# the3cloud/zktls

Hardware: AMD Instinct MI355X
Metric: trace-cells/s (higher is better)
Workload: dtype u32

## Files before the change

### include/zkhip.h

```cpp
#ifndef ZKHIP_H
#define ZKHIP_H
#include <stddef.h>
#include <stdint.h>

#ifdef __cplusplus
extern "C" {
#endif

#define ZKHIP_VERSION 100

typedef enum {
    ZKHIP_OK = 0,
    ZKHIP_ERR_INVALID = -1,
    ZKHIP_ERR_NO_DEVICE = -2,
    ZKHIP_ERR_HIP = -3,
    ZKHIP_ERR_NOMEM = -4,
    ZKHIP_ERR_BUFFER = -5,
    ZKHIP_ERR_VERIFY = -6,
    ZKHIP_ERR_INTERNAL = -7
} zkhip_status;

typedef struct zkhip_ctx zkhip_ctx;

typedef struct {
// ... 12 lines not shown

int zkhip_version(void);
const char* zkhip_last_error(void);
int zkhip_device_count(void);
int zkhip_ctx_create(int device, void* stream, zkhip_ctx** out);
void zkhip_ctx_destroy(zkhip_ctx* ctx);
int zkhip_ctx_sync(zkhip_ctx* ctx);
int zkhip_set_wait_mode(int blocking, int device);
void* zkhip_ctx_stream(zkhip_ctx* ctx);

int zkhip_malloc(zkhip_ctx* ctx, size_t bytes, void** d_ptr);
int zkhip_free(zkhip_ctx* ctx, void* d_ptr);
int zkhip_memcpy_h2d(zkhip_ctx* ctx, void* d_dst, const void* h_src, size_t bytes);
int zkhip_memcpy_d2h(zkhip_ctx* ctx, void* h_dst, const void* d_src, size_t bytes);
int zkhip_to_monty(zkhip_ctx* ctx, const uint32_t* d_in, uint32_t* d_out, size_t n);
int zkhip_from_monty(zkhip_ctx* ctx, const uint32_t* d_in, uint32_t* d_out, size_t n);

int zkhip_fill_uniform(zkhip_ctx* ctx, uint64_t seed, int log_n, uint32_t width,
                       uint32_t* d_out, size_t ld);
int zkhip_gen_trace(zkhip_ctx* ctx, uint64_t seed, uint64_t shard, int log_n, uint32_t width,
                    uint32_t* d_out, size_t ld);

int zkhip_gen_trace_logup(zkhip_ctx* ctx, uint64_t seed, uint64_t shard, int log_n, uint32_t width,
                          int pairs, uint32_t* d_out, size_t ld);

int zkhip_gen_trace_logup_cross(zkhip_ctx* ctx, uint64_t seed, uint64_t shard, uint64_t partner_shard, int log_n, uint32_t width,
                                uint32_t partner_width, int pairs, uint32_t* d_out, size_t ld);

int zkhip_dft(zkhip_ctx* ctx, const uint32_t* d_in, size_t in_ld, uint32_t* d_out, size_t out_ld,
              int log_n, uint32_t width, int inverse, int bitrev_out);
int zkhip_coset_lde(zkhip_ctx* ctx, const uint32_t* d_in, size_t in_ld, uint32_t* d_out,
                    size_t out_ld, int log_n, uint32_t width, int log_blowup, uint32_t shift);
int zkhip_ctx_set_lde_fusion(zkhip_ctx* ctx, int on);

int zkhip_commit(zkhip_ctx* ctx, const uint32_t* d_trace, size_t ld, int log_n, uint32_t width, int log_blowup,
                 int hash_width, uint32_t* d_lde, uint32_t* d_tree, uint32_t root[8]);

int zkhip_poseidon2_permute(zkhip_ctx* ctx, uint32_t* d_states, size_t count);
int zkhip_hash_rows(zkhip_ctx* ctx, const uint32_t* const* d_mats, const size_t* lds,
                    const uint32_t* widths, int nmats, size_t height, uint32_t* d_digests);
int zkhip_merkle_commit(zkhip_ctx* ctx, const uint32_t* const* d_mats, const size_t* lds,
                        const uint32_t* widths, int nmats, int log_h, uint32_t* d_tree);

int zkhip_merkle_commit_mixed(zkhip_ctx* ctx, const uint32_t* const* d_mats, const size_t* lds,
                              const uint32_t* widths, const int* log_heights, int nmats, uint32_t* d_tree);


int zkhip_quotient_values(zkhip_ctx* ctx, const uint32_t* d_lde, size_t ld, int log_n,
                          uint32_t width, const uint32_t alpha[4] ,
                          uint32_t* d_out);
int zkhip_perm_trace(zkhip_ctx* ctx, const uint32_t* d_trace, size_t ld, int log_n, uint32_t width, int pairs,
                     const uint32_t gamma[4], const uint32_t beta[4], uint32_t* d_out);
int zkhip_open_at(zkhip_ctx* ctx, const uint32_t* d_lde, size_t ld, int log_n, int log_blowup,
                  uint32_t width, const uint32_t* z, int npoints, uint32_t* h_out);
int zkhip_fri_fold(zkhip_ctx* ctx, const uint32_t* d_in, int log_h,
                   const uint32_t beta[4] , uint32_t* d_out);

int zkhip_fri_fold_k(zkhip_ctx* ctx, const uint32_t* d_in, int log_h, int log_arity,
                     const uint32_t beta[4] , uint32_t* d_out);

size_t zkhip_proof_size(int log_n, uint32_t width, const zkhip_params* prm, size_t n_public);
int zkhip_prove_shard(zkhip_ctx* ctx, const uint32_t* d_trace, size_t ld, int log_n,
                      uint32_t width, const uint32_t* public_values, size_t n_public,
                      const zkhip_params* prm, uint8_t* proof, size_t cap, size_t* len);
int zkhip_prove_shard_host(zkhip_ctx* ctx, const uint32_t* h_trace, int log_n, uint32_t width,
                           const uint32_t* public_values, size_t n_public, const zkhip_params* prm,
// ... 222 lines not shown
```

### zktls_amd/_lib.py

```python
import ctypes as C
import os

import numpy as np

P = 2013265921
_HERE = os.path.dirname(os.path.abspath(__file__))
LIB_PATH = os.path.join(_HERE, "libzkhip.so")

u32p = C.POINTER(C.c_uint32)
u8p = C.POINTER(C.c_uint8)

EXPORTS = [
    "zkhip_version", "zkhip_last_error", "zkhip_device_count", "zkhip_ctx_create", "zkhip_ctx_destroy",
    "zkhip_ctx_sync", "zkhip_ctx_set_lde_fusion", "zkhip_ctx_stream", "zkhip_malloc", "zkhip_free", "zkhip_memcpy_h2d",
    "zkhip_memcpy_d2h", "zkhip_to_monty", "zkhip_from_monty", "zkhip_fill_uniform", "zkhip_gen_trace",
    "zkhip_gen_trace_logup", "zkhip_gen_trace_logup_cross", "zkhip_perm_trace",
    "zkhip_dft", "zkhip_coset_lde", "zkhip_ntt_pass", "zkhip_poseidon2_permute", "zkhip_hash_rows",
    "zkhip_merkle_commit", "zkhip_merkle_commit_mixed", "zkhip_merkle_commit_p24_colmajor", "zkhip_batch_interpolate_colmajor", "zkhip_batch_expand_colmajor", "zkhip_quotient_values", "zkhip_open_at", "zkhip_fri_fold", "zkhip_fri_fold_k",
    "zkhip_commit", "zkhip_proof_size", "zkhip_prove_shard", "zkhip_prove_shard_host", "zkhip_prove_shards", "zkhip_prove_shards_multi", "zkhip_shard_device", "zkhip_release_cached_contexts", "zkhip_prove_segment", "zkhip_verify_shard", "zkhip_last_prove_debug",
    "zkhip_chips_proof_size", "zkhip_prove_chips", "zkhip_verify_chips", "zkhip_request_digest",
    "zkhip_eltwise_add", "zkhip_eltwise_copy", "zkhip_eltwise_zeroize", "zkhip_eltwise_sum_ext", "zkhip_zk_shift", "zkhip_mix_poly_coeffs",
    "zkhip_batch_evaluate_any", "zkhip_gather_sample", "zkhip_scatter", "zkhip_prefix_products_ext", "zkhip_hash_rows_sha256",
    "zkhip_hash_fold_sha256", "zkhip_merkle_commit_sha256_colmajor",
    "zkhip_bincode_size", "zkhip_proof_to_bincode", "zkhip_proof_from_bincode",
    "zkhip_chips_bincode_size", "zkhip_chips_proof_to_bincode", "zkhip_chips_proof_from_bincode",
    "zkhip_load_poseidon2_params", "zkhip_reset_poseidon2_params", "zkhip_poseidon2_params_name",
    "zkhip_air_validate", "zkhip_air_digest", "zkhip_air_synthetic", "zkhip_proof_size_air", "zkhip_prove_shard_air", "zkhip_verify_shard_air",
    "zkhip_quotient_values_air",
    "zkhip_chips_proof_size_air", "zkhip_prove_chips_air", "zkhip_verify_chips_air",
    "zkhip_prove_shards_air_multi", "zkhip_selftest_host_simd", "zkhip_host_permutation_ns", "zkhip_host_simd", "zkhip_recursion_witnesses_on_host", "zkhip_machine_proof_size", "zkhip_prove_machine", "zkhip_verify_machine", "zkhip_range_table",
    "zkhip_machine_setup", "zkhip_machine_key_destroy", "zkhip_machine_proof_size_keyed", "zkhip_prove_machine_keyed", "zkhip_verify_machine_keyed", "zkhip_prove_machine_keyed_at",
    "zkhip_sha256_setup", "zkhip_sha256_machine_proof_size", "zkhip_prove_sha256_machine", "zkhip_verify_sha256_machine", "zkhip_prove_transcripts", "zkhip_prove_transcripts_air", "zkhip_sha256_machine_describe", "zkhip_machine_verifier_setup", "zkhip_machine_verifier_key_host", "zkhip_machine_verifier_proof_size", "zkhip_prove_machine_verifier", "zkhip_prove_shard_tree", "zkhip_verify_machine_recursive", "zkhip_machine_verifier_describe", "zkhip_machine_verifier_host_tables", "zkhip_sha256_compress_setup", "zkhip_sha256_compress_key_host", "zkhip_sha256_compressed_proof_size", "zkhip_prove_sha256_compressed", "zkhip_verify_sha256_compressed", "zkhip_set_wait_mode", "zkhip_set_lockstep", "zkhip_lockstep_stats", "zkhip_lockstep_stack_high_water", "zkhip_set_fri_graph", "zkhip_shard_verifier_setup", "zkhip_shard_verifier_proof_size", "zkhip_shard_verifier_max_proofs", "zkhip_prove_shard_verifier", "zkhip_prove_shard_verifier_batch", "zkhip_verify_shard_recursive", "zkhip_shard_verifier_describe", "zkhip_shard_verifier_key_host", "zkhip_machine_key_host", "zkhip_shard_verifier_setup_air", "zkhip_shard_verifier_key_host_air", "zkhip_shard_verifier_max_proofs_air", "zkhip_shard_verifier_proof_size_air", "zkhip_prove_shard_verifier_air", "zkhip_verify_shard_recursive_air", "zkhip_shard_verifier_describe_air", "zkhip_poseidon2_params_generation", "zkhip_selftest_lockstep",
    "zkhip_sha256_air_chained", "zkhip_sha256_gen_trace_chained", "zkhip_sha256_sharded_count", "zkhip_sha256_shard_proof_size", "zkhip_prove_sha256_sharded",
    "zkhip_verify_sha256_sharded",
    "zkhip_fri_view_shard", "zkhip_fri_chip_width", "zkhip_fri_chip_air",
    
    "zkhip_fri_view_path_words", "zkhip_fri_view_shard_paths", "zkhip_fri_view_transcript", "zkhip_fri_layers_chip_air", "zkhip_p2chip_air_fri_layers",
    
    "zkhip_fri_transcript_chip_air", "zkhip_p2chip_air_fri_transcript",
    
    "zkhip_fri_indices_program", "zkhip_fri_indices_key", "zkhip_fri_indices_proof_size", "zkhip_prove_fri_indices", "zkhip_verify_fri_indices",
    "zkhip_prove_fri_indices_batch", "zkhip_fri_view_all",
    "zkhip_p2chip_air", "zkhip_p2chip_gen_merkle_trace", "zkhip_merkle_paths_proof_size", "zkhip_prove_merkle_paths", "zkhip_verify_merkle_paths",
    "zkhip_p24chip_air", "zkhip_p24chip_gen_merkle_trace", "zkhip_merkle_paths_p24_proof_size", "zkhip_prove_merkle_paths_p24", "zkhip_verify_merkle_paths_p24",
    "zkhip_sha256_air", "zkhip_sha256_digest", "zkhip_sha256_pad", "zkhip_sha256_padding_publics", "zkhip_sha256_gen_trace", "zkhip_sha256_proof_size", "zkhip_prove_sha256", "zkhip_verify_sha256",
]

# ... 39 lines not shown
                ("n_public", C.c_size_t), ("proof", u8p), ("proof_cap", C.c_size_t), ("proof_len", C.c_size_t), ("status", C.c_int32)]


class ProveDebug(C.Structure):
    _fields_ = [
        ("trace_root", C.c_uint32 * 8),
        ("quotient_root", C.c_uint32 * 8),
        ("alpha", C.c_uint32 * 4),
        ("zeta", C.c_uint32 * 4),
        ("fri_alpha", C.c_uint32 * 4),
        ("pow_witness", C.c_uint32),
    ]


_LIB = None


def load():
    global _LIB
    if _LIB is not None:
        return _LIB
    if not os.path.exists(LIB_PATH):
        raise ImportError("libzkhip.so not built: run `python -c 'import __graft_entry__ as g; g.build()'` "
                          "(zktls_amd has no CPU fallback)")
    L = C.CDLL(LIB_PATH)
    L.zkhip_last_error.restype = C.c_char_p
    L.zkhip_ctx_stream.restype = C.c_void_p
    L.zkhip_ctx_stream.argtypes = [C.c_void_p]
    L.zkhip_ctx_create.argtypes = [C.c_int, C.c_void_p, C.POINTER(C.c_void_p)]
    L.zkhip_ctx_destroy.argtypes = [C.c_void_p]
    L.zkhip_ctx_destroy.restype = None
    L.zkhip_ctx_sync.argtypes = [C.c_void_p]
    L.zkhip_ctx_set_lde_fusion.argtypes = [C.c_void_p, C.c_int]
    L.zkhip_malloc.argtypes = [C.c_void_p, C.c_size_t, C.POINTER(C.c_void_p)]
    L.zkhip_free.argtypes = [C.c_void_p, C.c_void_p]
    L.zkhip_memcpy_h2d.argtypes = [C.c_void_p, C.c_void_p, C.c_void_p, C.c_size_t]
    L.zkhip_memcpy_d2h.argtypes = [C.c_void_p, C.c_void_p, C.c_void_p, C.c_size_t]
    L.zkhip_to_monty.argtypes = [C.c_void_p, C.c_void_p, C.c_void_p, C.c_size_t]
    L.zkhip_from_monty.argtypes = [C.c_void_p, C.c_void_p, C.c_void_p, C.c_size_t]
    L.zkhip_fill_uniform.argtypes = [C.c_void_p, C.c_uint64, C.c_int, C.c_uint32, C.c_void_p, C.c_size_t]
    L.zkhip_gen_trace.argtypes = [C.c_void_p, C.c_uint64, C.c_uint64, C.c_int, C.c_uint32, C.c_void_p, C.c_size_t]
    L.zkhip_gen_trace_logup.argtypes = [C.c_void_p, C.c_uint64, C.c_uint64, C.c_int, C.c_uint32, C.c_int, C.c_void_p, C.c_size_t]
    L.zkhip_perm_trace.argtypes = [C.c_void_p, C.c_void_p, C.c_size_t, C.c_int, C.c_uint32, C.c_int, u32p, u32p, C.c_void_p]
    L.zkhip_dft.argtypes = [C.c_void_p, C.c_void_p, C.c_size_t, C.c_void_p, C.c_size_t, C.c_int, C.c_uint32, C.c_int, C.c_int]
    L.zkhip_coset_lde.argtypes = [C.c_void_p, C.c_void_p, C.c_size_t, C.c_void_p, C.c_size_t, C.c_int, C.c_uint32, C.c_int, C.c_uint32]
    L.zkhip_ntt_pass.argtypes = [C.c_void_p, C.c_void_p, C.c_void_p, C.c_size_t, C.c_int, C.c_uint32, C.c_int]
    L.zkhip_poseidon2_permute.argtypes = [C.c_void_p, C.c_void_p, C.c_size_t]
    L.zkhip_hash_rows.argtypes = [C.c_void_p, C.POINTER(C.c_void_p), C.POINTER(C.c_size_t), C.POINTER(C.c_uint32), C.c_int, C.c_size_t, C.c_void_p]
    L.zkhip_merkle_commit.argtypes = [C.c_void_p, C.POINTER(C.c_void_p), C.POINTER(C.c_size_t), C.POINTER(C.c_uint32), C.c_int, C.c_int, C.c_void_p]
    L.zkhip_merkle_commit_mixed.argtypes = [C.c_void_p, C.POINTER(C.c_void_p), C.POINTER(C.c_size_t), C.POINTER(C.c_uint32), C.POINTER(C.c_int), C.c_int, C.c_void_p]
    L.zkhip_merkle_commit_p24_colmajor.argtypes = [C.c_void_p, C.c_void_p, C.c_uint32, C.c_int, C.c_void_p]
    L.zkhip_batch_interpolate_colmajor.argtypes = [C.c_void_p, C.c_void_p, C.c_void_p, C.c_uint32, C.c_int]
    L.zkhip_batch_expand_colmajor.argtypes = [C.c_void_p, C.c_void_p, C.c_void_p, C.c_uint32, C.c_int, C.c_int, C.c_uint32]
    L.zkhip_quotient_values.argtypes = [C.c_void_p, C.c_void_p, C.c_size_t, C.c_int, C.c_uint32, u32p, C.c_void_p]
    L.zkhip_open_at.argtypes = [C.c_void_p, C.c_void_p, C.c_size_t, C.c_int, C.c_int, C.c_uint32, u32p, C.c_int, u32p]
    L.zkhip_fri_fold.argtypes = [C.c_void_p, C.c_void_p, C.c_int, u32p, C.c_void_p]
    L.zkhip_fri_fold_k.argtypes = [C.c_void_p, C.c_void_p, C.c_int, C.c_int, u32p, C.c_void_p]
    L.zkhip_proof_size.restype = C.c_size_t
    L.zkhip_proof_size.argtypes = [C.c_int, C.c_uint32, C.POINTER(Params), C.c_size_t]
    L.zkhip_prove_shard.argtypes = [C.c_void_p, C.c_void_p, C.c_size_t, C.c_int, C.c_uint32, u32p, C.c_size_t,
                                    C.POINTER(Params), u8p, C.c_size_t, C.POINTER(C.c_size_t)]
    L.zkhip_commit.argtypes = [C.c_void_p, C.c_void_p, C.c_size_t, C.c_int, C.c_uint32, C.c_int, C.c_int, C.c_void_p, C.c_void_p, u32p]
    L.zkhip_prove_shard_host.argtypes = [C.c_void_p, C.c_void_p, C.c_int, C.c_uint32, u32p, C.c_size_t,
                                         C.POINTER(Params), u8p, C.c_size_t, C.POINTER(C.c_size_t)]
    L.zkhip_release_cached_contexts.restype = None
    L.zkhip_prove_shards.argtypes = [C.c_int, C.POINTER(ShardJob), C.c_int, C.POINTER(Params), C.c_int, C.c_int]
# ... 229 lines not shown
```

### zktls_amd/csrc/context.cpp

```cpp
#include "context.h"
#include "poseidon2.cuh"

#include <atomic>
#include <mutex>
#include <vector>

#include <cstdio>
#include <cstdlib>
#include <cstring>
#include <string>

namespace zk {

extern std::atomic<int> g_live_contexts;

static thread_local std::string g_last_error;

void set_error(const std::string& msg) { g_last_error = msg; }
void fiber_tls_swap_error(std::string& err) { g_last_error.swap(err); }
int fail(int code, const std::string& msg) { g_last_error = msg; return code; }
int hip_fail(hipError_t e, const char* what) {
    g_last_error = std::string("HIP error ") + hipGetErrorName(e) + " (" + hipGetErrorString(e) + ") in " + what;
    (void)hipGetLastError();
    return e == hipErrorOutOfMemory ? ZKHIP_ERR_NOMEM : ZKHIP_ERR_HIP;
// ... 490 lines not shown
    void* coef_v;
    ZK_TRY(ctx_reserve(ctx, S_COEF, n * width * 4, &coef_v));
    uint32_t* coef = (uint32_t*)coef_v;
    const uint32_t wnb = two_adic_generator(log_n + log_blowup);
    if (m1 == 0) {
        ZK_TRY(run_inverse(ctx, in, in_ld, coef, width, log_n, width, false));
        for (int t = 0; t < B; t++) {
            const uint32_t st = fmul(shift, fpow(wnb, (uint64_t)t));
            uint32_t* dst = out + (size_t)reverse_bits((uint32_t)t, log_blowup) * n * out_ld;
            const NttPlan* p;
            ZK_TRY(get_plan(ctx, log_n, 1, st, &p));
            NttPassArgs a = base_args(ctx, coef, width, dst, out_ld, width, false);
            a.num_tiles = 1; a.log_m = log_n; a.in_tile_mul = 0; a.in_stride = 1; a.out_tile_mul = 0; a.out_stride = 1;
            a.pre = p->pre; a.bitrev_out = 1;
            ZK_HIP(launch_ntt_pass(a, false, ctx->stream));
        }
        return ZKHIP_OK;
    }
    uint32_t* dsts[16];
    uint32_t shifts[16];
    for (int t = 0; t < B; t++) {
        shifts[t] = fmul(shift, fpow(wnb, (uint64_t)t));
        dsts[t] = out + (size_t)reverse_bits((uint32_t)t, log_blowup) * n * out_ld;
    }
    return lde_two_pass(ctx, in, in_ld, coef, width, dsts, out_ld, log_n, width, shifts, B);
}

int op_merkle_commit(zkhip_ctx* ctx, const MatDesc* mats, int nmats, int log_h, uint32_t* tree) {
    if (nmats < 1 || nmats > MAX_LEAF_MATS) return fail(ZKHIP_ERR_INVALID, "merkle_commit: 1..8 matrices");
    if (log_h < 0 || log_h > 30) return fail(ZKHIP_ERR_INVALID, "merkle_commit: bad log_h");
    LeafArgs la{};
    for (int m = 0; m < nmats; m++) la.mats[m] = mats[m];
    la.nmats = nmats; la.height = (uint64_t)1 << log_h; la.digests = tree;
    uint32_t* level = tree;
    uint64_t count = la.height;
    if (count > COOP_TOP_NODES && count <= coop_max_nodes()) {
        const uint32_t rest = count >= 4096 ? 128u : 32u;
        ZK_HIP(launch_hash_sub(la, (uint32_t)count / rest, ctx->stream));
        for (uint64_t c = count; c > rest; c >>= 1) level += 8 * c;
        ZK_HIP(launch_compress_top(level, rest, ctx->stream));
        return ZKHIP_OK;
    }
    ZK_HIP(launch_hash_rows(la, ctx->stream));
    while (count > COOP_TOP_NODES) {
        if (count <= coop_max_nodes()) {
            const uint32_t rest = count >= 4096 ? 128u : 32u;
            const uint32_t sub = (uint32_t)count / rest;
            ZK_HIP(launch_compress_sub(level, (uint32_t)count, sub, ctx->stream));
            for (uint64_t c = count; c > rest; c >>= 1) level += 8 * c;
            count = rest;
            break;
        }
        uint32_t* next = level + 8 * count;
        ZK_HIP(launch_compress_level(level, next, count / 2, ctx->stream));
        level = next; count >>= 1;
    }
    ZK_HIP(launch_compress_top(level, (uint32_t)count, ctx->stream));
    return ZKHIP_OK;
}

int op_merkle_commit_mixed(zkhip_ctx* ctx, const MatDesc* mats, const int* log_heights, int nmats, uint32_t* tree) {
    if (nmats < 1 || nmats > 32) return fail(ZKHIP_ERR_INVALID, "merkle_commit_mixed: 1..32 matrices");
    int log_h = 0;
    for (int m = 0; m < nmats; m++) {
        if (log_heights[m] < 0 || log_heights[m] > 30) return fail(ZKHIP_ERR_INVALID, "merkle_commit_mixed: bad height");
        if (log_heights[m] > log_h) log_h = log_heights[m];
// ... 110 lines not shown
    }
    const int logical = device;
#ifdef ZKHIP_AB_HOOKS
    if (logical_devices() > 0) {
        if (device < 0 || device >= logical_devices()) return fail(ZKHIP_ERR_INVALID, "ctx_create: logical device ordinal out of range");
        device = physical_device(device);
    }
#endif
    if (device < 0 || device >= n) return fail(ZKHIP_ERR_INVALID, "ctx_create: device ordinal out of range");
    ZK_HIP(hipSetDevice(device));
    hipDeviceProp_t prop;
    ZK_HIP(hipGetDeviceProperties(&prop, device));
    if (std::strncmp(prop.gcnArchName, "gfx950", 6) != 0)
        return fail(ZKHIP_ERR_NO_DEVICE, std::string("device is ") + prop.gcnArchName + ", libzkhip is built for gfx950 only");
    zkhip_ctx* ctx = new (std::nothrow) zkhip_ctx();
    if (!ctx) return fail(ZKHIP_ERR_NOMEM, "ctx_create: out of host memory");
    g_live_contexts.fetch_add(1);
    ctx->device = device;
    ctx->logical_device = logical;
    if (stream) { ctx->stream = (hipStream_t)stream; ctx->own_stream = false; }
    else {
        hipError_t e = hipStreamCreateWithFlags(&ctx->stream, hipStreamNonBlocking);
        if (e != hipSuccess) { delete ctx; g_live_contexts.fetch_sub(1); return hip_fail(e, "hipStreamCreate"); }
        ctx->own_stream = true;
    }
    int rc = ZKHIP_OK;
    do {
        hipError_t e;
        if ((e = hipMalloc((void**)&ctx->w1024_fwd, 1024 * 4)) != hipSuccess) { rc = hip_fail(e, "hipMalloc"); break; }
        if ((e = hipMalloc((void**)&ctx->w1024_inv, 1024 * 4)) != hipSuccess) { rc = hip_fail(e, "hipMalloc"); break; }
        const uint32_t w = two_adic_generator(10);
        if ((e = launch_pow_table(ctx->w1024_fwd, 1024, w, MONTY_R1, ctx->stream)) != hipSuccess) { rc = hip_fail(e, "pow_table"); break; }
        if ((e = launch_pow_table(ctx->w1024_inv, 1024, finv(w), MONTY_R1, ctx->stream)) != hipSuccess) { rc = hip_fail(e, "pow_table"); break; }
        if ((e = hipMalloc((void**)&ctx->w1024f_fwd, 1024 * 4)) != hipSuccess) { rc = hip_fail(e, "hipMalloc"); break; }
        if ((e = hipMalloc((void**)&ctx->w1024f_inv, 1024 * 4)) != hipSuccess) { rc = hip_fail(e, "hipMalloc"); break; }
        if ((e = launch_fused_table(ctx->w1024f_fwd, ctx->w1024_fwd, 1, 0, ctx->stream)) != hipSuccess) { rc = hip_fail(e, "fused_table"); break; }
        if ((e = launch_fused_table(ctx->w1024f_inv, ctx->w1024_inv, 1, 0, ctx->stream)) != hipSuccess) { rc = hip_fail(e, "fused_table"); break; }
        if ((e = hash_upload_p2_tables(g_p2_tables, ctx->stream)) != hipSuccess) { rc = hip_fail(e, "upload Poseidon2 tables"); break; }
        if ((e = stark_upload_p2_tables(g_p2_tables, ctx->stream)) != hipSuccess) { rc = hip_fail(e, "upload Poseidon2 tables"); break; }
        if ((e = hipStreamSynchronize(ctx->stream)) != hipSuccess) { rc = hip_fail(e, "sync"); break; }
    } while (0);
    if (rc != ZKHIP_OK) { zkhip_ctx_destroy(ctx); return rc; }
    *out = ctx;
    return ZKHIP_OK;
}

void zkhip_ctx_destroy(zkhip_ctx* ctx) {
    if (!ctx) return;
    (void)hipSetDevice(ctx->device);
    if (ctx->stream) (void)hipStreamSynchronize(ctx->stream);
    if (ctx->sha_key) zkhip_machine_key_destroy(ctx->sha_key);
    if (ctx->rec_key) zkhip_machine_key_destroy(ctx->rec_key);
    if (ctx->fri_graph_exec) (void)hipGraphExecDestroy(ctx->fri_graph_exec);
    for (NttPlan& p : ctx->plans) { if (p.pre) (void)hipFree(p.pre); if (p.post) (void)hipFree(p.post); if (p.pre_f) (void)hipFree(p.pre_f); if (p.post_f) (void)hipFree(p.post_f); }
    if (ctx->w1024f_fwd) (void)hipFree(ctx->w1024f_fwd);
    if (ctx->w1024f_inv) (void)hipFree(ctx->w1024f_inv);
    for (BigPlan& p : ctx->big_plans) if (p.tw) (void)hipFree(p.tw);
    for (SmallPlan& p : ctx->small_plans) { if (p.tw_inv) (void)hipFree(p.tw_inv); if (p.tw_fwd) (void)hipFree(p.tw_fwd); }
    for (SmallPre& p : ctx->small_pres) if (p.pre) (void)hipFree(p.pre);
    for (ColPlan& p : ctx->col_plans) { if (p.pre) (void)hipFree(p.pre); if (p.post2d) (void)hipFree(p.post2d); }
    for (DeviceBuffer& b : ctx->scratch) if (b.ptr) (void)hipFree(b.ptr);
    if (ctx->host_pinned) (void)hipHostFree(ctx->host_pinned);
    if (ctx->w1024_fwd) (void)hipFree(ctx->w1024_fwd);
    if (ctx->w1024_inv) (void)hipFree(ctx->w1024_inv);
    for (auto& d : ctx->domains) { (void)hipFree(d.xs); (void)hipFree(d.sel_first); (void)hipFree(d.sel_last); (void)hipFree(d.itw); }
    if (ctx->own_stream && ctx->stream) (void)hipStreamDestroy(ctx->stream);
    delete ctx;
    g_live_contexts.fetch_sub(1);
}

#define CHECK_CTX(ctx)                                                  \
    do {                                                                \
        if (!(ctx)) return fail(ZKHIP_ERR_INVALID, "null context");     \
        ZK_HIP(hipSetDevice((ctx)->device));                            \
    } while (0)

int zkhip_ctx_set_lde_fusion(zkhip_ctx* ctx, int on) {
    CHECK_CTX(ctx);
    const int prev = ctx->lde_fusion ? 1 : 0;
    ctx->lde_fusion = on != 0;
    return prev;
}
int zkhip_ctx_sync(zkhip_ctx* ctx) { CHECK_CTX(ctx); return dev_sync(ctx); }
int zkhip_set_wait_mode(int blocking, int device) {
    int n = 0;
    if (hipGetDeviceCount(&n) != hipSuccess || n <= 0) { (void)hipGetLastError(); return fail(ZKHIP_ERR_NO_DEVICE, "set_wait_mode: no HIP device visible"); }
    if (device >= n) return fail(ZKHIP_ERR_INVALID, "set_wait_mode: no such device");
    if (g_live_contexts.load() != 0) return fail(ZKHIP_ERR_INVALID, "set_wait_mode: contexts exist (the mode is fixed when a device is first used)");
    int cur = 0;
    (void)hipGetDevice(&cur);
    int rc = ZKHIP_OK;
    for (int d = device < 0 ? 0 : device; d < (device < 0 ? n : device + 1); d++) {
        hipError_t e = hipSetDevice(d);
        if (e == hipSuccess) e = hipSetDeviceFlags(blocking ? hipDeviceScheduleBlockingSync : hipDeviceScheduleAuto);
        if (e != hipSuccess) { (void)hipGetLastError(); rc = hip_fail(e, "hipSetDeviceFlags (too late: the device is already in use?)"); }
    }
    (void)hipSetDevice(device < 0 ? cur : device);
    return rc;
}
void* zkhip_ctx_stream(zkhip_ctx* ctx) { return ctx ? (void*)ctx->stream : nullptr; }

int zkhip_malloc(zkhip_ctx* ctx, size_t bytes, void** d_ptr) {
    CHECK_CTX(ctx);
    if (!d_ptr) return fail(ZKHIP_ERR_INVALID, "malloc: null out pointer");
    ZK_HIP(hipMalloc(d_ptr, bytes ? bytes : 4));
#ifdef ZKHIP_AB_HOOKS
    if (logical_devices() > 0) { std::lock_guard<std::mutex> lk(g_alloc_mu); g_allocs.push_back({{(uintptr_t)*d_ptr, bytes ? bytes : 4}, ctx->logical_device}); }
#endif
    return ZKHIP_OK;
}
int zkhip_free(zkhip_ctx* ctx, void* d_ptr) {
    CHECK_CTX(ctx);
    ZK_HIP(hipStreamSynchronize(ctx->stream));
// ... 295 lines not shown
```

### zktls_amd/csrc/context.h

```cpp
#pragma once
#include <hip/hip_runtime.h>

#include <deque>
#include <functional>
#include <new>
#include <string>
#include <vector>

#include "../../include/zkhip.h"
#include "../../include/zkhip_chips.h"
#include "../../include/zkhip_hal.h"
#include "babybear.cuh"
#include "kernels.h"

namespace zk {

void set_error(const std::string& msg);
int fail(int code, const std::string& msg);
int hip_fail(hipError_t e, const char* what);

#define ZK_HIP(call)                                            \
    do {                                                        \
        hipError_t _e = (call);                                 \
        if (_e != hipSuccess) return zk::hip_fail(_e, #call);   \
// ... 60 lines not shown
    S_STAGE,
    S_RO,
    S_EXTRA_A, S_EXTRA_B,
    S_CTREE,
    S_CHIP,
    S_LOOKUP,
    S_ADDEND,
    S_CHIP_B,
    S_KEYTRACE,
    S_REC_A, S_REC_B, S_REC_C, S_REC_D, S_REC_E, S_REC_F, S_REC_G, S_REC_H, S_REC_I, S_REC_J,
    S_WIT_A, S_WIT_B, S_WIT_C,
    S_COUNT
};

}

struct zkhip_ctx {
    int device = 0;
    int logical_device = 0;
    hipStream_t stream = nullptr;
    bool own_stream = false;
    uint32_t* w1024_fwd = nullptr;
    uint32_t* w1024_inv = nullptr;
    uint32_t* w1024f_fwd = nullptr;
    uint32_t* w1024f_inv = nullptr;
    std::deque<zk::NttPlan> plans;
    std::deque<zk::BigPlan> big_plans;
    std::deque<zk::SmallPlan> small_plans;
    std::deque<zk::SmallPre> small_pres;
    std::deque<zk::ColPlan> col_plans;
    zk::DeviceBuffer scratch[zk::S_COUNT];
    zkhip_prove_debug debug{};
    bool lde_fusion = true;
    struct DomainSet { int log_n, log_blowup; uint32_t *xs, *sel_first, *sel_last, *itw; };
    std::vector<DomainSet> domains;
    int dom_log_n = -1, dom_log_blowup = 0;
    uint32_t* dom_xs = nullptr;
    uint32_t* dom_sel_first = nullptr;
    uint32_t* dom_sel_last = nullptr;
    uint32_t* dom_itw = nullptr;
    std::vector<uint64_t> fri_graph_key;
    hipGraphExec_t fri_graph_exec = nullptr;
    zkhip_machine_key* sha_key = nullptr;
    int sha_key_blowup = 0;
    uint32_t sha_vk[8] = {0};
    zkhip_machine_key* rec_key = nullptr;
    std::vector<uint64_t> rec_key_sig;
    uint32_t rec_vk[8] = {0};
    void* host_pinned = nullptr;
    size_t host_pinned_bytes = 0;
};

namespace zk {
constexpr int MAX_LOG_ROWS = 22;
int ctx_reserve(zkhip_ctx* ctx, int slot, size_t bytes, void** out);
int ctx_host_pinned(zkhip_ctx* ctx, size_t bytes, void** out);
extern thread_local int t_query_threads_cap;
int fri_view_all_unhashed(const uint8_t* proof, size_t len, int log_n, uint32_t width, const uint32_t* public_values, size_t n_public, const zkhip_params* prm,
                          uint32_t* betas, uint32_t final_value[4], uint32_t* indices, uint32_t* values, uint32_t* siblings, uint32_t* roots, uint32_t* paths,
                          uint32_t transcript[10], const uint32_t* program = nullptr, size_t program_words = 0);
int get_plan(zkhip_ctx* ctx, int log_n, int kind, uint32_t shift_monty, const NttPlan** out);
int op_coset_lde(zkhip_ctx* ctx, const uint32_t* d_in, size_t in_ld, uint32_t* d_out, size_t out_ld,
                 int log_n, uint32_t width, int log_blowup, uint32_t shift_monty);
int op_merkle_commit(zkhip_ctx* ctx, const MatDesc* mats, int nmats, int log_h, uint32_t* d_tree);
int op_merkle_commit_mixed(zkhip_ctx* ctx, const MatDesc* mats, const int* log_heights, int nmats, uint32_t* d_tree);
int deal_jobs(const int* devices, int n_devices, int n_jobs, int in_flight, const std::function<int(zkhip_ctx*, int)>& run, std::vector<char>& ran);
// ... 31 lines not shown
```

### zktls_amd/csrc/hash.hip

```cpp
#include "poseidon2.cuh"
#include "kernels.h"
#include "batch.h"
#include "p24chip.h"
#include "p2chip.h"

namespace zk {

hipError_t hash_upload_p2_tables(const P2Tables& t, hipStream_t s) { return p2_upload_tables(t, s); }

__device__ __forceinline__ uint32_t load_virtual(const LeafArgs& a, uint64_t row, uint32_t vc) {
    uint32_t off = vc;
#pragma unroll
    for (int m = 0; m < MAX_LEAF_MATS; m++) {
        if (m < a.nmats) {
            if (off < a.mats[m].width) return a.mats[m].ptr[row * a.mats[m].ld + off];
            off -= a.mats[m].width;
        }
    }
    return 0u;
}

__global__ void hash_rows16_kernel(LeafArgs a, uint32_t total_w);
struct hash_rows16_kernel_bargs { LeafArgs a; uint32_t total_w; static hash_rows16_kernel_bargs make(LeafArgs a, uint32_t total_w) { return hash_rows16_kernel_bargs{a, total_w}; } };
__global__ void hash_rows16_kernel_batch(const hash_rows16_kernel_bargs* __restrict__ zk_arr);
// ... 348 lines not shown
    __syncthreads();
    uint32_t* level = a.digests;
    uint32_t n = (uint32_t)a.height, mine = sub;
    while (mine > 1) {
        uint32_t* next = level + 8 * (size_t)n;
        const size_t in0 = (size_t)blockIdx.x * mine, out0 = (size_t)blockIdx.x * (mine / 2);
        for (uint32_t i = grp; i < mine / 2; i += ngrp) {
            const uint32_t x = coop_permute(level[16 * (in0 / 2 + i) + lane16], lane16, k);
            if (lane16 < 8) next[8 * (out0 + i) + lane16] = x;
        }
        __threadfence_block();
        __syncthreads();
        level = next; n >>= 1; mine >>= 1;
    }
}
__global__ void __launch_bounds__(1024) hash_sub16_kernel(LeafArgs a, uint32_t total_w, uint32_t sub) { hash_sub16_kernel_body(a, total_w, sub); }
__global__ void __launch_bounds__(1024) hash_sub16_kernel_batch(const hash_sub16_kernel_bargs* __restrict__ zk_arr) { const hash_sub16_kernel_bargs& zk_b = zk_arr[blockIdx.z]; hash_sub16_kernel_body(zk_b.a, zk_b.total_w, zk_b.sub); }

__device__ __forceinline__ void hash_rows16_kernel_body(const LeafArgs& a, uint32_t total_w) {
    const uint32_t gid = blockIdx.x * blockDim.x + threadIdx.x;
    const uint64_t row = gid >> 4;
    const int lane16 = threadIdx.x & 15;
    if (row >= a.height) return;
    const CoopConsts k = coop_load_consts(lane16);
    uint32_t x = 0;
    for (uint32_t q = 0; q < total_w; q += 8) {
        if (lane16 < 8 && q + lane16 < total_w) x = load_virtual(a, row, q + lane16);
        x = coop_permute(x, lane16, k);
    }
    if (lane16 < 8) a.digests[row * 8 + lane16] = x;
}
__global__ void __launch_bounds__(256) hash_rows16_kernel(LeafArgs a, uint32_t total_w) { hash_rows16_kernel_body(a, total_w); }
__global__ void __launch_bounds__(256) hash_rows16_kernel_batch(const hash_rows16_kernel_bargs* __restrict__ zk_arr) { const hash_rows16_kernel_bargs& zk_b = zk_arr[blockIdx.z]; hash_rows16_kernel_body(zk_b.a, zk_b.total_w); }


ZK_D void chal_observe_root_sample_ext(uint32_t& x, int& n_in, int& n_out, uint32_t* sin, uint32_t* sout, int lane, const CoopConsts& k,
                                       const uint32_t* root, uint32_t* beta_out, uint32_t* root_log) {
    auto duplex = [&]() {
        if (lane < n_in) x = sin[lane];
        n_in = 0;
        x = coop_permute(x, lane, k);
        if (lane < 8) sout[lane] = x;
        n_out = 8;
    };
    for (int w = 0; w < 8; w++) {
        const uint32_t v = root[w];
        if (lane == 0 && root_log) root_log[w] = v;
        n_out = 0;
        if (lane == 0) sin[n_in] = v;
        n_in++;
        if (n_in == 8) duplex();
    }
    for (int e = 0; e < 4; e++) {
        if (n_in != 0 || n_out == 0) duplex();
        --n_out;
        if (lane == 0) beta_out[e] = sout[n_out];
    }
}
__device__ __forceinline__ void fri_challenge_kernel_body(DevChallenger* c, const uint32_t* __restrict__ root, uint32_t* __restrict__ beta_out, uint32_t* __restrict__ root_log) {
    __shared__ uint32_t sin[8], sout[8];
    const int lane = threadIdx.x;
    if (lane >= 16) return;
    const CoopConsts k = coop_load_consts(lane);
    uint32_t x = c->state[lane];
    int n_in = c->n_in, n_out = c->n_out;
    if (lane < 8) { sin[lane] = c->in[lane]; sout[lane] = c->out[lane]; }
// ... 824 lines not shown
```

### zktls_amd/csrc/kernels.h

```cpp
#pragma once
#include <hip/hip_runtime.h>
#include <stddef.h>
#include <stdint.h>

#include "babybear.cuh"

namespace zk {

struct NttPassArgs {
    const uint32_t* in;
    uint32_t* out;
    uint64_t in_ld, out_ld;
    uint32_t ncols;
    uint32_t num_tiles;
    uint32_t log_m;
    uint64_t in_tile_mul, in_stride;
    uint64_t out_tile_mul, out_stride;
    uint32_t bitrev_out;
    uint32_t map_mode;
    uint64_t tile_perm;
    uint32_t fast_path;
    uint32_t debug_flags;
    uint32_t cols_per_thread;
    uint32_t bench_tag;
// ... 65 lines not shown
    const uint32_t* tw;
};
hipError_t launch_ntt_combine(const CombineArgs& a, hipStream_t s);
hipError_t launch_combine_table(uint32_t* out, uint32_t rows, uint64_t groups, uint32_t w, uint32_t shift, uint32_t scale, int bits, hipStream_t s);

hipError_t launch_pow_table(uint32_t* out, size_t n, uint32_t base, uint32_t scale, hipStream_t s);
hipError_t launch_post_table(uint32_t* out, uint32_t rows, uint32_t cols, uint32_t omega,
                             uint32_t shift, uint32_t scale, hipStream_t s);

struct MatDesc {
    const uint32_t* ptr;
    uint64_t ld;
    uint32_t width;
};
constexpr int MAX_LEAF_MATS = 8;
constexpr uint32_t COOP_MAX_NODES = 16384;
uint32_t coop_max_nodes();
constexpr uint32_t COOP_TOP_NODES = 512;
struct LeafArgs {
    MatDesc mats[MAX_LEAF_MATS];
    int nmats;
    uint64_t height;
    uint32_t* digests;
};
hipError_t launch_hash_rows(const LeafArgs& a, hipStream_t s);
hipError_t launch_compress_level(const uint32_t* children, uint32_t* parents, uint64_t count,
                                 hipStream_t s);
hipError_t launch_inject(uint32_t* nodes, const uint32_t* extra, uint64_t count, hipStream_t s);
bool compress_inject_ok(const LeafArgs& a);
hipError_t launch_compress_inject(const uint32_t* children, const LeafArgs& a, hipStream_t s);
hipError_t launch_compress_top(uint32_t* tree, uint32_t count, hipStream_t s);
hipError_t launch_compress_sub(uint32_t* tree, uint32_t count, uint32_t sub, hipStream_t s);
hipError_t launch_hash_sub(const LeafArgs& a, uint32_t sub, hipStream_t s);
hipError_t launch_merkle_p24_colmajor(const uint32_t* mat, uint32_t cols, int log_rows, uint32_t* tree, hipStream_t s);
hipError_t launch_merkle_p24_rowmajor(const uint32_t* mat, uint64_t ld, uint32_t width, int log_rows, uint32_t* tree, hipStream_t s);
struct P2Tables;
hipError_t hash_upload_p2_tables(const P2Tables& t, hipStream_t s);
hipError_t stark_upload_p2_tables(const P2Tables& t, hipStream_t s);
namespace p2chip { struct MerkleTraceArgs; struct LayerPathsArgs; struct P2RArgs; struct MrecChainArgs; }
hipError_t launch_p2chip_merkle(const p2chip::MerkleTraceArgs& a, hipStream_t s);
namespace p24chip { struct MerkleTraceArgs; }
hipError_t launch_p24chip_merkle(const p24chip::MerkleTraceArgs& a, hipStream_t s);
hipError_t launch_p2chip_layer_paths(const p2chip::LayerPathsArgs& a, hipStream_t s);
hipError_t launch_mrec_chains(const p2chip::MrecChainArgs& a, hipStream_t s);
hipError_t launch_p2r_rows(const p2chip::P2RArgs& a, hipStream_t s);
hipError_t launch_permute_states(uint32_t* states, uint64_t count, hipStream_t s);

hipError_t launch_fill_uniform(uint32_t* out, uint64_t ld, uint64_t seed, uint64_t rows,
                               uint32_t width, hipStream_t s);
hipError_t launch_gen_trace(uint32_t* out, uint64_t ld, uint64_t seed, uint64_t rows,
                            uint32_t width, hipStream_t s);
hipError_t launch_gen_trace_logup(uint32_t* out, uint64_t ld, uint64_t seed, uint64_t rows, uint32_t width, uint32_t pairs,
                                  uint64_t recv_seed, uint32_t recv_width, hipStream_t s);
hipError_t launch_small_eval(const uint32_t* in, uint64_t in_ld, uint32_t* out, uint64_t out_ld, int log_n, int log_out, uint32_t width,
                             uint32_t w, uint32_t shift, uint32_t scale, int bitrev_out, hipStream_t s);
hipError_t launch_transpose(const uint32_t* in, uint32_t* out, uint64_t rows, uint64_t cols, int rev_bits_in, int rev_bits_out, hipStream_t s);
hipError_t launch_convert(const uint32_t* in, uint32_t* out, uint64_t n, bool to_monty_form,
                          hipStream_t s);

hipError_t launch_domain_tables(uint32_t* xs, uint32_t* sel_first, uint32_t* sel_last, uint32_t* itw, int log_n, int log_blowup, hipStream_t s);

struct QuotientArgs {
    const uint32_t* lde;
    uint64_t ld;
    uint32_t width;
    int log_n;
// ... 158 lines not shown
```

### zktls_amd/csrc/prover.cpp

```cpp
#include <atomic>
#include <chrono>
#include <condition_variable>
#include <deque>
#include <cstring>
#include <functional>
#include <mutex>
#include <string>
#include <thread>
#include <vector>

#include "proof_common.h"
#include "batch.h"

namespace zk { std::atomic<bool> g_fri_graph{true}; }
namespace zk {

extern std::atomic<uint64_t> g_p2_generation;
void air_digest_cached(const AirView& a, uint32_t out[8]) {
    struct Entry { std::vector<uint32_t> words; uint64_t generation; uint32_t dg[8]; };
    static std::mutex mu;
    static std::vector<Entry> cache;
    const uint64_t gen = g_p2_generation.load();
    {
        std::lock_guard<std::mutex> lk(mu);
// ... 188 lines not shown
        uint32_t* tree = ltrees + tree_off[l];
        ZK_TRY(commit_hw(ctx, cur, 4 * arity, (uint32_t)(4 * arity), lh, tree, sh.hw));
        Ext beta = ext_zero();
        if (d_chal) {
            ZK_HIP(launch_fri_challenge(d_chal, tree + (2 * rows - 2) * 8, d_betas + 4 * l, d_roots + 8 * l, st));
        } else {
            ZK_TRY(d2h(ctx, root, tree + (2 * rows - 2) * 8, 32));
            for (int i = 0; i < 8; i++) { ch.observe(root[i]); pf[pos++] = from_monty(root[i]); }
            beta = ch.sample_ext();
        }
        const uint32_t* src = cur;
        for (int j = 0; j < K; j++) {
            const size_t out_cnt = (size_t)1 << (H - K * l - j - 1);
            uint32_t* dst = (j == K - 1) ? layers + layer_off[l + 1] : fold_tmp + ((j & 1) ? 4 * (m / 2) : 0);
            if (d_chal) ZK_HIP(launch_fri_fold_dev(src, dst, ctx->dom_itw, out_cnt, d_betas + 4 * l, j, st));
            else ZK_HIP(launch_fri_fold(src, dst, ctx->dom_itw, out_cnt, beta, st));
            src = dst;
            beta = ext_mul(beta, beta);
        }
        const int reached = H - K * (l + 1);
        if (inject && inject[reached]) ZK_HIP(launch_ext_add(layers + layer_off[l + 1], inject[reached], (uint64_t)1 << reached, st));
    }
    return ZKHIP_OK;
    };
#ifdef ZKHIP_AB_HOOKS
    static const bool env_graph = [] { const char* e = getenv("ZKHIP_FRI_GRAPH"); return !e || atoi(e) != 0; }();
    const bool use_graph = env_graph && g_fri_graph.load();
#else
    const bool use_graph = g_fri_graph.load();
#endif
    if (d_chal && use_graph && !t_batcher) {
        std::vector<uint64_t> key = {(uint64_t)H, (uint64_t)K, (uint64_t)RL, (uint64_t)sh.hw, (uint64_t)m, (uint64_t)(uintptr_t)layers,
                                     (uint64_t)(uintptr_t)ltrees, (uint64_t)(uintptr_t)fold_tmp, (uint64_t)(uintptr_t)d_chal,
                                     (uint64_t)(uintptr_t)ctx->dom_itw};
        for (size_t o : layer_off) key.push_back(o);
        for (size_t o : tree_off) key.push_back(o);
        if (inject) for (int h = 0; h <= H; h++) key.push_back((uint64_t)(uintptr_t)inject[h]);
        if (!ctx->fri_graph_exec || ctx->fri_graph_key != key) {
            if (ctx->fri_graph_exec) { (void)hipGraphExecDestroy(ctx->fri_graph_exec); ctx->fri_graph_exec = nullptr; }
            hipGraph_t graph = nullptr;
            ZK_HIP(hipStreamBeginCapture(st, hipStreamCaptureModeThreadLocal));
            const int rc = enqueue_layers();
            const hipError_t ce = hipStreamEndCapture(st, &graph);
            if (rc != ZKHIP_OK) { if (graph) (void)hipGraphDestroy(graph); return rc; }
            ZK_HIP(ce);
            const hipError_t ie = hipGraphInstantiate(&ctx->fri_graph_exec, graph, nullptr, nullptr, 0);
            (void)hipGraphDestroy(graph);
            ZK_HIP(ie);
            ctx->fri_graph_key = key;
        }
        ZK_HIP(hipGraphLaunch(ctx->fri_graph_exec, st));
    } else {
        ZK_TRY(enqueue_layers());
    }
    if (d_chal) {
        std::vector<uint32_t> log((size_t)RL * 12);
        ZK_TRY(d2h(ctx, log.data(), d_betas, log.size() * 4));
        for (int l = 0; l < RL; l++) {
            const uint32_t* r = log.data() + 4 * (size_t)RL + 8 * (size_t)l;
            for (int i = 0; i < 8; i++) { ch.observe(r[i]); pf[pos++] = from_monty(r[i]); }
            const Ext beta = ch.sample_ext();
            const uint32_t* b = log.data() + 4 * (size_t)l;
            if (beta.c[0] != b[0] || beta.c[1] != b[1] || beta.c[2] != b[2] || beta.c[3] != b[3])
                return fail(ZKHIP_ERR_INTERNAL, "prove: device and host transcripts disagree in the FRI commit phase");
        }
    }
    return ZKHIP_OK;
// ... 1143 lines not shown
```

### zktls_amd/device.py

```python
import ctypes as C
import weakref

import numpy as np

from . import _lib
from ._lib import Params, ProveDebug, check, from_monty, to_monty, u32p, u8p


SHA256_WIDTH, SHA256_PUBLIC, SHA256_PADDING_PUBLIC = 640, 91, 75


class DeviceBuffer:

    def __init__(self, ctx, nwords, ptr=None, owner=None):
        self.ctx = ctx
        self.nwords = int(nwords)
        self._owned = ptr is None
        self._owner = owner
        if ptr is None:
            p = C.c_void_p()
            check(ctx.lib.zkhip_malloc(ctx.handle, C.c_size_t(self.nwords * 4), C.byref(p)))
            ptr = p.value
            ctx._buffers.add(self)
        self.ptr = ptr
# ... 34 lines not shown

    def __init__(self, buf, words):
        self.base = buf
        self.ptr = buf.ptr + 4 * int(words)


class Context:
    def __init__(self, device=0, stream=None):
        self.lib = _lib.load()
        h = C.c_void_p()
        check(self.lib.zkhip_ctx_create(int(device), C.c_void_p(stream) if stream else None, C.byref(h)))
        self.handle = h
        self.device = device
        self._buffers = weakref.WeakSet()

    def close(self):
        if self.handle:
            for b in list(self._buffers):
                b.free()
            self.lib.zkhip_ctx_destroy(self.handle)
            self.handle = None

    def __del__(self):
        try:
            self.close()
        except Exception:
            pass

    def sync(self):
        check(self.lib.zkhip_ctx_sync(self.handle))

    def set_lde_fusion(self, on):
        r = self.lib.zkhip_ctx_set_lde_fusion(self.handle, 1 if on else 0)
        if r < 0:
            check(r)
        return bool(r)

    @property
    def stream(self):
        return self.lib.zkhip_ctx_stream(self.handle)

    def alloc(self, nwords):
        return DeviceBuffer(self, nwords)

    def wrap(self, tensor):
        return DeviceBuffer(self, tensor.numel(), ptr=tensor.data_ptr(), owner=tensor)

    def from_numpy(self, canonical):
        a = np.ascontiguousarray(canonical, dtype=np.uint32)
        buf = self.alloc(a.size)
        buf.upload(a)
        return buf

    def fill_uniform(self, seed, log_n, width, out=None):
        out = out or self.alloc(width << log_n)
        check(self.lib.zkhip_fill_uniform(self.handle, seed, log_n, width, C.c_void_p(out.ptr), width))
        return out

    def gen_trace_logup_cross(self, seed, shard, partner_shard, log_n, width, partner_width, pairs, out=None):
        out = out or self.alloc(width << log_n)
        check(self.lib.zkhip_gen_trace_logup_cross(self.handle, seed, shard, partner_shard, log_n, width, partner_width, pairs, C.c_void_p(out.ptr), width))
        return out

    def gen_trace(self, seed, shard, log_n, width, out=None):
        out = out or self.alloc(width << log_n)
        check(self.lib.zkhip_gen_trace(self.handle, seed, shard, log_n, width, C.c_void_p(out.ptr), width))
# ... 1375 lines not shown
```

Before: 19.92 billion.

## Fuse Merkle leaf hashing and tree climb into one kernel

Adds a kernel that hashes leaf rows and then climbs the Merkle tree inside the same launch. It uses a last-block-arrives atomic counter so the final workgroup in each group carries on to the upper levels. It is enabled by default for trees up to the cooperative size limit and replaces the multi-launch level-by-level path. The aim is to cut kernel launch overhead and inter-level synchronization, at the cost of serialized upper levels on few workgroups and reliance on atomic/fence correctness.

```diff
diff --git a/include/zkhip.h b/include/zkhip.h
--- a/include/zkhip.h
+++ b/include/zkhip.h
@@ -68,6 +68,8 @@
 int zkhip_coset_lde(zkhip_ctx* ctx, const uint32_t* d_in, size_t in_ld, uint32_t* d_out,
                     size_t out_ld, int log_n, uint32_t width, int log_blowup, uint32_t shift);
 int zkhip_ctx_set_lde_fusion(zkhip_ctx* ctx, int on);
+
+int zkhip_ctx_set_tree_fusion(zkhip_ctx* ctx, int on);
 
 int zkhip_commit(zkhip_ctx* ctx, const uint32_t* d_trace, size_t ld, int log_n, uint32_t width, int log_blowup,
                  int hash_width, uint32_t* d_lde, uint32_t* d_tree, uint32_t root[8]);
diff --git a/zktls_amd/_lib.py b/zktls_amd/_lib.py
--- a/zktls_amd/_lib.py
+++ b/zktls_amd/_lib.py
@@ -12,7 +12,7 @@
 
 EXPORTS = [
     "zkhip_version", "zkhip_last_error", "zkhip_device_count", "zkhip_ctx_create", "zkhip_ctx_destroy",
-    "zkhip_ctx_sync", "zkhip_ctx_set_lde_fusion", "zkhip_ctx_stream", "zkhip_malloc", "zkhip_free", "zkhip_memcpy_h2d",
+    "zkhip_ctx_sync", "zkhip_ctx_set_lde_fusion", "zkhip_ctx_set_tree_fusion", "zkhip_ctx_stream", "zkhip_malloc", "zkhip_free", "zkhip_memcpy_h2d",
     "zkhip_memcpy_d2h", "zkhip_to_monty", "zkhip_from_monty", "zkhip_fill_uniform", "zkhip_gen_trace",
     "zkhip_gen_trace_logup", "zkhip_gen_trace_logup_cross", "zkhip_perm_trace",
     "zkhip_dft", "zkhip_coset_lde", "zkhip_ntt_pass", "zkhip_poseidon2_permute", "zkhip_hash_rows",
@@ -118,6 +118,7 @@
     L.zkhip_ctx_destroy.restype = None
     L.zkhip_ctx_sync.argtypes = [C.c_void_p]
     L.zkhip_ctx_set_lde_fusion.argtypes = [C.c_void_p, C.c_int]
+    L.zkhip_ctx_set_tree_fusion.argtypes = [C.c_void_p, C.c_int]
     L.zkhip_malloc.argtypes = [C.c_void_p, C.c_size_t, C.POINTER(C.c_void_p)]
     L.zkhip_free.argtypes = [C.c_void_p, C.c_void_p]
     L.zkhip_memcpy_h2d.argtypes = [C.c_void_p, C.c_void_p, C.c_void_p, C.c_size_t]
diff --git a/zktls_amd/csrc/context.cpp b/zktls_amd/csrc/context.cpp
--- a/zktls_amd/csrc/context.cpp
+++ b/zktls_amd/csrc/context.cpp
@@ -546,6 +546,10 @@
     LeafArgs la{};
     for (int m = 0; m < nmats; m++) la.mats[m] = mats[m];
     la.nmats = nmats; la.height = (uint64_t)1 << log_h; la.digests = tree;
+    if (ctx->tree_fusion && la.height <= coop_max_nodes()) {
+        ZK_HIP(launch_merkle_tree(la, ctx->tree_ctr, ctx->stream));
+        return ZKHIP_OK;
+    }
     uint32_t* level = tree;
     uint64_t count = la.height;
     if (count > COOP_TOP_NODES && count <= coop_max_nodes()) {
@@ -722,6 +726,8 @@
         const uint32_t w = two_adic_generator(10);
         if ((e = launch_pow_table(ctx->w1024_fwd, 1024, w, MONTY_R1, ctx->stream)) != hipSuccess) { rc = hip_fail(e, "pow_table"); break; }
         if ((e = launch_pow_table(ctx->w1024_inv, 1024, finv(w), MONTY_R1, ctx->stream)) != hipSuccess) { rc = hip_fail(e, "pow_table"); break; }
+        if ((e = hipMalloc((void**)&ctx->tree_ctr, 16)) != hipSuccess) { rc = hip_fail(e, "hipMalloc"); break; }
+        if ((e = hipMemsetAsync(ctx->tree_ctr, 0, 16, ctx->stream)) != hipSuccess) { rc = hip_fail(e, "hipMemset"); break; }
         if ((e = hipMalloc((void**)&ctx->w1024f_fwd, 1024 * 4)) != hipSuccess) { rc = hip_fail(e, "hipMalloc"); break; }
         if ((e = hipMalloc((void**)&ctx->w1024f_inv, 1024 * 4)) != hipSuccess) { rc = hip_fail(e, "hipMalloc"); break; }
         if ((e = launch_fused_table(ctx->w1024f_fwd, ctx->w1024_fwd, 1, 0, ctx->stream)) != hipSuccess) { rc = hip_fail(e, "fused_table"); break; }
@@ -743,6 +749,7 @@
     if (ctx->rec_key) zkhip_machine_key_destroy(ctx->rec_key);
     if (ctx->fri_graph_exec) (void)hipGraphExecDestroy(ctx->fri_graph_exec);
     for (NttPlan& p : ctx->plans) { if (p.pre) (void)hipFree(p.pre); if (p.post) (void)hipFree(p.post); if (p.pre_f) (void)hipFree(p.pre_f); if (p.post_f) (void)hipFree(p.post_f); }
+    if (ctx->tree_ctr) (void)hipFree(ctx->tree_ctr);
     if (ctx->w1024f_fwd) (void)hipFree(ctx->w1024f_fwd);
     if (ctx->w1024f_inv) (void)hipFree(ctx->w1024f_inv);
     for (BigPlan& p : ctx->big_plans) if (p.tw) (void)hipFree(p.tw);
@@ -769,6 +776,12 @@
     CHECK_CTX(ctx);
     const int prev = ctx->lde_fusion ? 1 : 0;
     ctx->lde_fusion = on != 0;
+    return prev;
+}
+int zkhip_ctx_set_tree_fusion(zkhip_ctx* ctx, int on) {
+    CHECK_CTX(ctx);
+    const int prev = ctx->tree_fusion ? 1 : 0;
+    ctx->tree_fusion = on != 0;
     return prev;
 }
 int zkhip_ctx_sync(zkhip_ctx* ctx) { CHECK_CTX(ctx); return dev_sync(ctx); }
diff --git a/zktls_amd/csrc/context.h b/zktls_amd/csrc/context.h
--- a/zktls_amd/csrc/context.h
+++ b/zktls_amd/csrc/context.h
@@ -116,6 +116,8 @@
     zk::DeviceBuffer scratch[zk::S_COUNT];
     zkhip_prove_debug debug{};
     bool lde_fusion = true;
+    bool tree_fusion = true;
+    uint32_t* tree_ctr = nullptr;
     struct DomainSet { int log_n, log_blowup; uint32_t *xs, *sel_first, *sel_last, *itw; };
     std::vector<DomainSet> domains;
     int dom_log_n = -1, dom_log_blowup = 0;
diff --git a/zktls_amd/csrc/hash.hip b/zktls_amd/csrc/hash.hip
--- a/zktls_amd/csrc/hash.hip
+++ b/zktls_amd/csrc/hash.hip
@@ -404,6 +404,76 @@
 }
 __global__ void __launch_bounds__(256) hash_rows16_kernel(LeafArgs a, uint32_t total_w) { hash_rows16_kernel_body(a, total_w); }
 __global__ void __launch_bounds__(256) hash_rows16_kernel_batch(const hash_rows16_kernel_bargs* __restrict__ zk_arr) { const hash_rows16_kernel_bargs& zk_b = zk_arr[blockIdx.z]; hash_rows16_kernel_body(zk_b.a, zk_b.total_w); }
+
+__device__ __forceinline__ void tree_climb(uint32_t* level, uint32_t n, uint32_t mine, uint32_t* ctr, const CoopConsts& k) {
+    __shared__ uint32_t last;
+    const int lane16 = threadIdx.x & 15;
+    const uint32_t grp = threadIdx.x >> 4, ngrp = blockDim.x >> 4;
+    uint32_t b = blockIdx.x;
+    for (;;) {
+        asm volatile("s_waitcnt vmcnt(0)" ::: "memory");
+        __syncthreads();
+        while (mine > 1) {
+            uint32_t* next = level + 8 * (size_t)n;
+            const size_t in0 = (size_t)b * mine, out0 = (size_t)b * (mine / 2);
+            for (uint32_t i = grp; i < mine / 2; i += ngrp) {
+                const uint32_t x = coop_permute(level[16 * (in0 / 2 + i) + lane16], lane16, k);
+                if (lane16 < 8) next[8 * (out0 + i) + lane16] = x;
+            }
+            asm volatile("s_waitcnt vmcnt(0)" ::: "memory");
+            __syncthreads();
+            level = next; n >>= 1; mine >>= 1;
+        }
+        if (n == 1) return;
+        const uint32_t G = n < 2 * ngrp ? n : 2 * ngrp;
+        __attribute__((address_space(1))) uint32_t* c = (__attribute__((address_space(1))) uint32_t*)(ctr + b / G);
+        if (threadIdx.x == 0) {
+            __builtin_amdgcn_fence(__ATOMIC_RELEASE, "agent");
+            asm volatile("s_waitcnt vmcnt(0)" ::: "memory");
+            const bool l = __hip_atomic_fetch_add(c, 1u, __ATOMIC_RELAXED, __HIP_MEMORY_SCOPE_AGENT) == G - 1;
+            if (l) {
+                __hip_atomic_store(c, 0u, __ATOMIC_RELAXED, __HIP_MEMORY_SCOPE_AGENT);
+                __builtin_amdgcn_fence(__ATOMIC_ACQUIRE, "agent");
+                asm volatile("s_waitcnt vmcnt(0)" ::: "memory");
+            }
+            last = l ? 1u : 0u;
+        }
+        __syncthreads();
+        if (!last) return;
+        ctr += n / G; b /= G; mine = G;
+    }
+}
+
+__device__ __forceinline__ void hash_tree16_kernel_body(const LeafArgs& a, uint32_t total_w, uint32_t sub, uint32_t* ctr) {
+    const int lane16 = threadIdx.x & 15;
+    const uint32_t grp = threadIdx.x >> 4, ngrp = blockDim.x >> 4;
+    const CoopConsts k = coop_load_consts(lane16);
+    for (uint32_t i = grp; i < sub; i += ngrp) {
+        const uint64_t row = (uint64_t)blockIdx.x * sub + i;
+        uint32_t x = 0;
+        for (uint32_t q = 0; q < total_w; q += 8) {
+            if (lane16 < 8 && q + lane16 < total_w) x = load_virtual(a, row, q + lane16);
+            x = coop_permute(x, lane16, k);
+        }
+        if (lane16 < 8) a.digests[row * 8 + lane16] = x;
+    }
+    tree_climb(a.digests, (uint32_t)a.height, sub, ctr, k);
+}
+__global__ void __launch_bounds__(1024) hash_tree16_kernel(LeafArgs a, uint32_t total_w, uint32_t sub, uint32_t* ctr) { hash_tree16_kernel_body(a, total_w, sub, ctr); }
+struct hash_tree16_kernel_bargs { LeafArgs a; uint32_t total_w; uint32_t sub; uint32_t* ctr; static hash_tree16_kernel_bargs make(LeafArgs a, uint32_t total_w, uint32_t sub, uint32_t* ctr) { return hash_tree16_kernel_bargs{a, total_w, sub, ctr}; } };
+__global__ void __launch_bounds__(1024) hash_tree16_kernel_batch(const hash_tree16_kernel_bargs* __restrict__ zk_arr) { const hash_tree16_kernel_bargs& zk_b = zk_arr[blockIdx.z]; hash_tree16_kernel_body(zk_b.a, zk_b.total_w, zk_b.sub, zk_b.ctr); }
+
+hipError_t launch_merkle_tree(const LeafArgs& a, uint32_t* ctr, hipStream_t s) {
+    const uint64_t h = a.height;
+    if (h == 0 || (h & (h - 1)) || h > coop_max_nodes() || a.nmats < 1 || a.nmats > MAX_LEAF_MATS) return hipErrorInvalidValue;
+    uint32_t total = 0;
+    for (int m = 0; m < a.nmats; m++) total += a.mats[m].width;
+    const uint32_t nwg = h >= 4096 ? 128u : h > 512 ? 32u : h >= 64 ? (uint32_t)h / 64 : 1u;
+    const uint32_t sub = (uint32_t)h / nwg;
+    const unsigned threads = nwg > 1 ? 1024u : (sub * 16 < 64 ? 64u : sub * 16);
+    ZK_LAUNCH(hash_tree16_kernel, hash_tree16_kernel_batch, hash_tree16_kernel_bargs, dim3(nwg), dim3(threads), 0, s, a, total, sub, ctr);
+    return hipGetLastError();
+}
 
 
 ZK_D void chal_observe_root_sample_ext(uint32_t& x, int& n_in, int& n_out, uint32_t* sin, uint32_t* sout, int lane, const CoopConsts& k,
diff --git a/zktls_amd/csrc/kernels.h b/zktls_amd/csrc/kernels.h
--- a/zktls_amd/csrc/kernels.h
+++ b/zktls_amd/csrc/kernels.h
@@ -121,6 +121,7 @@
 hipError_t launch_compress_top(uint32_t* tree, uint32_t count, hipStream_t s);
 hipError_t launch_compress_sub(uint32_t* tree, uint32_t count, uint32_t sub, hipStream_t s);
 hipError_t launch_hash_sub(const LeafArgs& a, uint32_t sub, hipStream_t s);
+hipError_t launch_merkle_tree(const LeafArgs& a, uint32_t* ctr, hipStream_t s);
 hipError_t launch_merkle_p24_colmajor(const uint32_t* mat, uint32_t cols, int log_rows, uint32_t* tree, hipStream_t s);
 hipError_t launch_merkle_p24_rowmajor(const uint32_t* mat, uint64_t ld, uint32_t width, int log_rows, uint32_t* tree, hipStream_t s);
 struct P2Tables;
diff --git a/zktls_amd/csrc/prover.cpp b/zktls_amd/csrc/prover.cpp
--- a/zktls_amd/csrc/prover.cpp
+++ b/zktls_amd/csrc/prover.cpp
@@ -244,7 +244,7 @@
     if (d_chal && use_graph && !t_batcher) {
         std::vector<uint64_t> key = {(uint64_t)H, (uint64_t)K, (uint64_t)RL, (uint64_t)sh.hw, (uint64_t)m, (uint64_t)(uintptr_t)layers,
                                      (uint64_t)(uintptr_t)ltrees, (uint64_t)(uintptr_t)fold_tmp, (uint64_t)(uintptr_t)d_chal,
-                                     (uint64_t)(uintptr_t)ctx->dom_itw};
+                                     (uint64_t)(uintptr_t)ctx->dom_itw, (uint64_t)ctx->tree_fusion};
         for (size_t o : layer_off) key.push_back(o);
         for (size_t o : tree_off) key.push_back(o);
         if (inject) for (int h = 0; h <= H; h++) key.push_back((uint64_t)(uintptr_t)inject[h]);
diff --git a/zktls_amd/device.py b/zktls_amd/device.py
--- a/zktls_amd/device.py
+++ b/zktls_amd/device.py
@@ -90,6 +90,12 @@
 
     def set_lde_fusion(self, on):
         r = self.lib.zkhip_ctx_set_lde_fusion(self.handle, 1 if on else 0)
+        if r < 0:
+            check(r)
+        return bool(r)
+
+    def set_tree_fusion(self, on):
+        r = self.lib.zkhip_ctx_set_tree_fusion(self.handle, 1 if on else 0)
         if r < 0:
             check(r)
         return bool(r)
```

New measurement: 19.69 billion (median of 2 runs). Within noise of the previous version (-1.2%).
